# XChenZ/havatar

Hardware: AMD Instinct MI355X
Metric: rendered frames/sec @512^2, 64 samples/ray (higher is better)
Workload: dtype f32 emulated, full-width operands: every operand = hi + lo fp16 + tail (= the fp32 value itself, >= 24 significant bits); the three leading partial products on v_mfma_f32_32x32x16_f16, the three terms of order 2^-22 (hi.tail, tail.hi, lo.lo) on block-scaled 4-/6-bit v_mfma_scale_f32_32x32x64_f8f6f4

## Files before the change

### havatar_amd/csrc/hav_render.hip

```cpp
#include "hav_common.h"
#include <stdio.h>
#include <stdlib.h>
#include <string.h>
#include <atomic>

#define HAV_HID 128
#define HAV_PC 64
#define HAV_IN (2 * HAV_PC + 48)
#define KPE_STEPS 24
#define K2_STEPS (HAV_HID / 2)
#define OFF_W1PE 0
#define OFF_W2 (OFF_W1PE + KPE_STEPS * 4 * 64)
#define OFF_W4 (OFF_W2 + K2_STEPS * 4 * 64)
#define OFF_WFT (OFF_W4 + K2_STEPS * 2 * 4)
#define LDS_FLOATS (OFF_WFT + HAV_HID * 64)
#define OFF_B1 LDS_FLOATS
#define OFF_B2 (OFF_B1 + 128)
#define OFF_B4 (OFF_B2 + 128)
#define OFF_BF (OFF_B4 + 4)
#define OFF_W1F (OFF_BF + 64)
#define OFF_WFF (OFF_W1F + 2 * 128 * 64)
#define OFF_A1S (OFF_WFF + K2_STEPS * 2 * 64)
#define OFF_A2S (OFF_A1S + 3 * 4 * 3 * 64 * 4)
#define OFF_W4S (OFF_A2S + 8 * 4 * 3 * 64 * 4)
// ... 704 lines not shown
            float v[8];
            if (c < nc) getv(4 * g + c, v);
            else {
#pragma unroll
                for (int e = 0; e < 8; ++e) v[e] = 0.f;
            }
#pragma unroll
            for (int q = 0; q < 4; ++q) {
                typedef float f2 __attribute__((ext_vector_type(2)));
                typedef _Float16 h2 __attribute__((ext_vector_type(2)));
                const float v0 = v[2 * q], v1 = v[2 * q + 1];
                const h2 hi = __builtin_convertvector(f2{v0, v1}, h2);
                const uint32_t ph = __builtin_bit_cast(uint32_t, hi);
                float d0, d1;
                asm("v_fma_mix_f32 %0, %1, -1.0, %2 op_sel:[0,0,0] op_sel_hi:[1,0,0]" : "=v"(d0) : "v"(ph), "v"(v0));
                asm("v_fma_mix_f32 %0, %1, -1.0, %2 op_sel:[1,0,0] op_sel_hi:[1,0,0]" : "=v"(d1) : "v"(ph), "v"(v1));
                const h2 lo = __builtin_convertvector(f2{d0, d1}, h2);
                const uint32_t pl = __builtin_bit_cast(uint32_t, lo);
                float t0, t1;
                asm("v_fma_mix_f32 %0, %1, -1.0, %2 op_sel:[0,0,0] op_sel_hi:[1,0,0]" : "=v"(t0) : "v"(pl), "v"(d0));
                asm("v_fma_mix_f32 %0, %1, -1.0, %2 op_sel:[1,0,0] op_sel_hi:[1,0,0]" : "=v"(t1) : "v"(pl), "v"(d1));
                if (q == 0) { xh4[c].x = ph; xl4[c].x = pl; } else if (q == 1) { xh4[c].y = ph; xl4[c].y = pl; }
                else if (q == 2) { xh4[c].z = ph; xl4[c].z = pl; } else { xh4[c].w = ph; xl4[c].w = pl; }
                TB[4 * c + q] = __builtin_amdgcn_perm(__float_as_uint(t1), __float_as_uint(t0), 0x07060302u);
                if (DYN) vmax = fmaxf(vmax, fmaxf(fabsf(v0), fabsf(v1)));
            }
        }
        unsigned int E = DYN ? (__float_as_uint(vmax) >> 23) : 127u;
        if (DYN) E = E < 40u ? 40u : (E > 254u ? 254u : E);
        const unsigned int bh = E - 3u, bl = E - 13u, bt = (E - 26u) < 98u ? 98u : (E - 26u);
        const float sch = __uint_as_float(bh << 23), scl = __uint_as_float(bl << 23), sct = __uint_as_float(bt << 23);
        const int sbv = (int)(bh | (bl << 8) | (bt << 16));
        typedef _Float16 f16x16_t __attribute__((ext_vector_type(16)));
        auto cat32 = [](const uint4 (&x)[4]) {
            const f16x16_t a = __builtin_shufflevector(__builtin_bit_cast(f16x8_t, x[0]), __builtin_bit_cast(f16x8_t, x[1]), 0, 1, 2, 3, 4, 5, 6, 7, 8, 9, 10, 11, 12, 13, 14, 15);
            const f16x16_t b = __builtin_shufflevector(__builtin_bit_cast(f16x8_t, x[2]), __builtin_bit_cast(f16x8_t, x[3]), 0, 1, 2, 3, 4, 5, 6, 7, 8, 9, 10, 11, 12, 13, 14, 15);
            return __builtin_shufflevector(a, b, 0, 1, 2, 3, 4, 5, 6, 7, 8, 9, 10, 11, 12, 13, 14, 15, 16, 17, 18, 19, 20, 21, 22, 23, 24, 25, 26, 27, 28, 29, 30, 31);
        };
        const u32x6_t H6 = __builtin_amdgcn_cvt_scalef32_pk32_bf6_f16(cat32(xh4), sch);
        const u32x6_t L6 = __builtin_amdgcn_cvt_scalef32_pk32_fp6_f16(cat32(xl4), scl);
        const u32x6_t T6 = __builtin_amdgcn_cvt_scalef32_pk32_bf6_bf16(__builtin_bit_cast(bf16x32_t, TB), sct);
        const unsigned int* rec = mx + g * 4 * MX_G_DWORDS;
        u32x4_t ah[2], at[2], ala[2]; u32x2_t alb[2]; int sc[2];
        auto ldrec = [&](int slot, int m) {
            const unsigned int* r = rec + m * MX_G_DWORDS;
            ah[slot] = reinterpret_cast<const u32x4_t*>(r)[lane];
            at[slot] = reinterpret_cast<const u32x4_t*>(r + 256)[lane];
            ala[slot] = reinterpret_cast<const u32x4_t*>(r + 512)[lane];
            alb[slot] = reinterpret_cast<const u32x2_t*>(r + 768)[lane];
            sc[slot] = (int)r[896 + lane];
        };
        ldrec(0, 0);
#pragma unroll
        for (int m = 0; m < 4; ++m) {
            if (m + 1 < 4) ldrec((m + 1) & 1, m + 1);
            const int k = m & 1;
            if (HAV_MX_TERMS & 1) acc[m] = __builtin_amdgcn_mfma_scale_f32_32x32x64_f8f6f4(mx_op4(ah[k]), mx_op6(T6), acc[m], 4, 3, 0, sc[k], 2, sbv);
            if (HAV_MX_TERMS & 2) acc[m] = __builtin_amdgcn_mfma_scale_f32_32x32x64_f8f6f4(mx_op4(at[k]), mx_op6(H6), acc[m], 4, 3, 1, sc[k], 0, sbv);
            if (HAV_MX_TERMS & 4) acc[m] = __builtin_amdgcn_mfma_scale_f32_32x32x64_f8f6f4(mx_op6(ala[k], alb[k]), mx_op6(L6), acc[m], 2, 2, 2, sc[k], 1, sbv);
        }
        uint4 A[2][2];
#pragma unroll
        for (int q = 0; q < 2; ++q) A[0][q] = frag[((4 * g * 4) * 2 + q) * 64 + lane];
#pragma unroll
        for (int gg = 0; gg < 16; ++gg) {
            const int c = gg >> 2, m = gg & 3;
            if (c < nc) {
                const f16x8_t xh = __builtin_bit_cast(f16x8_t, xh4[c]), xl = __builtin_bit_cast(f16x8_t, xl4[c]);
                const f16x8_t ahh = __builtin_bit_cast(f16x8_t, A[gg & 1][0]), all_ = __builtin_bit_cast(f16x8_t, A[gg & 1][1]);
                acc[m] = __builtin_amdgcn_mfma_f32_32x32x16_f16(all_, xh, acc[m], 0, 0, 0);
                if (gg + 1 < 4 * nc) {
#pragma unroll
                    for (int q = 0; q < 2; ++q) A[(gg + 1) & 1][q] = frag[(((4 * g) * 4 + gg + 1) * 2 + q) * 64 + lane];
                }
                acc[m] = __builtin_amdgcn_mfma_f32_32x32x16_f16(ahh, xl, acc[m], 0, 0, 0);
                acc[m] = __builtin_amdgcn_mfma_f32_32x32x16_f16(ahh, xh, acc[m], 0, 0, 0);
            }
        }
    }
}

#include "hav_render_lab.h"

template <int GQ, int PREC, bool BLK, bool LEAN = false, typename Cont>
__device__ __forceinline__ void sample_eval(const MarchArgs& a_in, const LaneCtx& L, int b, float ox, float oy, float oz, float dx,
                                            float dy, float dz, float z, Cont&& cont PROF_ARG DBG_ARG)
{
    const MarchArgs& a = a_in;
    int lane = L.lane;
    asm volatile("" : "+v"(lane));
    const int h = lane >> 5;
    const float* sW1 = L.sW1;
    const float* sW2 = L.sW2;
    const float4* sW4 = L.sW4;
    int sb_off = 0;
    asm volatile("" : "+v"(sb_off));
    const float4* sBt = L.sB + sb_off;
    const int PR = a.p.plane_res, VR = a.p.vol_res;
    const float px = ox + dx * z, py = oy + dy * z, pz = oz + dz * z;
    const float* iT = a.inv_T + (size_t)b * 12;
    const float tx_ = px + iT[9], ty_ = py + iT[10], tz_ = pz + iT[11];
    const float p1x = tx_ * iT[0] + ty_ * iT[3] + tz_ * iT[6];
    const float p1y = tx_ * iT[1] + ty_ * iT[4] + tz_ * iT[7];
    const float p1z = tx_ * iT[2] + ty_ * iT[5] + tz_ * iT[8];
    float wmine;
    {
        const float gx = (h ? p1x : px) * a.p.skin_scale[0] + a.p.skin_trans[0];
        const float gy = (h ? p1y : py) * a.p.skin_scale[1] + a.p.skin_trans[1];
        const float gz = (h ? p1z : pz) * a.p.skin_scale[2] + a.p.skin_trans[2];
        const float lim = a.vlim;
        float ix = ((gx + 1.0f) * 0.5f) * lim, iy = ((gy + 1.0f) * 0.5f) * lim, iz = ((gz + 1.0f) * 0.5f) * lim;
        ix = fminf(fmaxf(ix, 0.f), lim); iy = fminf(fmaxf(iy, 0.f), lim); iz = fminf(fmaxf(iz, 0.f), lim);
        const float x0f = floorf(ix), y0f = floorf(iy), z0f = floorf(iz);
        const float fx = ix - x0f, fy = iy - y0f, fz = iz - z0f;
        const int x0 = (int)x0f, y0 = (int)y0f, z0 = (int)z0f;
        const int x1 = min(x0 + 1, VR - 1), y1 = min(y0 + 1, VR - 1), z1 = min(z0 + 1, VR - 1);
        const float* v = a.vol + (size_t)h * VR * VR * VR;
        float acc = 0.f;
#pragma unroll
        for (int cz = 0; cz < 2; ++cz)
#pragma unroll
            for (int cy = 0; cy < 2; ++cy)
#pragma unroll
                for (int cx = 0; cx < 2; ++cx) {
                    const float wgt = (cx ? fx : 1.0f - fx) * (cy ? fy : 1.0f - fy) * (cz ? fz : 1.0f - fz);
                    acc += v[((size_t)(cz ? z1 : z0) * VR + (cy ? y1 : y0)) * VR + (cx ? x1 : x0)] * wgt;
                }
        wmine = acc;
    }
    const float wother = half_swap(wmine, h);
    const float w0 = h ? wother : wmine, w1 = h ? wmine : wother;
    const float den = (w0 + w1) + 1e-8f;
    float rden = __builtin_amdgcn_rcpf(den);
    rden = rden * (2.0f - den * rden);
    float n0 = w0 * rden, n1 = w1 * rden;
    const float qx_ = n0 * px + n1 * p1x, qy_ = n0 * py + n1 * p1y, qz_ = n0 * pz + n1 * p1z;
    DBG_PUT(4, z); DBG_PUT(5, wmine); DBG_PUT(6, wother); DBG_PUT(7, (qx_ + qy_) + qz_);
    DBG_PUT(8, den); DBG_PUT(9, n0); DBG_PUT(10, n1); DBG_PUT(11, (px + py + pz) + (p1x + p1y + p1z));
    TICK(1);

    auto bias_init = [&](f32x16 (&acc1)[4]) {
#pragma unroll
        for (int m = 0; m < 4; ++m)
#pragma unroll
            for (int q = 0; q < 4; ++q) {
                if (BLK) {
                    const float4 bl = sBt[8 * m + 2 * q + h];
                    acc1[m][4 * q + 0] = bl.x; acc1[m][4 * q + 1] = bl.y; acc1[m][4 * q + 2] = bl.z; acc1[m][4 * q + 3] = bl.w;
                    continue;
                }
                const auto bb = LDB4(OFF_B1 + 32 * m + 8 * q);
                acc1[m][4 * q + 0] = __uint_as_float(bb[0]); acc1[m][4 * q + 1] = __uint_as_float(bb[1]);
                acc1[m][4 * q + 2] = __uint_as_float(bb[2]); acc1[m][4 * q + 3] = __uint_as_float(bb[3]);
            }
    };
    auto gather = [&](f32x16 (&acc1)[4]) {
        if (!ABL(1)) {
            const float lim = a.plim;
            const float gy = qy_ * a.p.nerf_scale[1] + a.p.nerf_trans[1];
            const float iy = ((gy + 1.0f) * 0.5f) * lim;
            float y0f = floorf(iy);
            const float wy1 = iy - y0f, wy0 = 1.0f - wy1;
            y0f = fminf(fmaxf(y0f, -2.f), lim + 2.f);
            const int y0 = (int)y0f, y1 = y0 + 1;
            const bool vy0 = y0 >= 0 && y0 < PR, vy1 = y1 >= 0 && y1 < PR;
            const int cy0 = min(max(y0, 0), PR - 1), cy1 = min(max(y1, 0), PR - 1);
            float tw[8];
            const float4* tp[8];
#pragma unroll
            for (int pl = 0; pl < 2; ++pl) {
                const float gx = pl ? qz_ * a.p.nerf_scale[2] + a.p.nerf_trans[2] : qx_ * a.p.nerf_scale[0] + a.p.nerf_trans[0];
                const float ix = ((gx + 1.0f) * 0.5f) * lim;
                float x0f = floorf(ix);
                const float wx1 = ix - x0f, wx0 = 1.0f - wx1;
                x0f = fminf(fmaxf(x0f, -2.f), lim + 2.f);
                const int x0 = (int)x0f, x1 = x0 + 1;
                const bool vx0 = x0 >= 0 && x0 < PR, vx1 = x1 >= 0 && x1 < PR;
                const int cx0 = min(max(x0, 0), PR - 1), cx1 = min(max(x1, 0), PR - 1);
                tw[4 * pl + 0] = (vx0 && vy0) ? wx0 * wy0 : 0.f; tw[4 * pl + 1] = (vx1 && vy0) ? wx1 * wy0 : 0.f;
                tw[4 * pl + 2] = (vx0 && vy1) ? wx0 * wy1 : 0.f; tw[4 * pl + 3] = (vx1 && vy1) ? wx1 * wy1 : 0.f;
                const int tg = pl ? HAV_TG1 : HAV_TG;
                const float* plb = a.pplanes + ((size_t)pl * a.p.B + b) * PR * PR * 128 + h * (64 << tg);
                auto texel = [&](int cy, int cx) { return reinterpret_cast<const float4*>(plb + ((size_t)((cy * PR + cx) >> tg)) * (128 << tg) + (cx & ((1 << tg) - 1)) * 4); };
                tp[4 * pl + 0] = texel(cy0, cx0);
                tp[4 * pl + 1] = texel(cy0, cx1);
                tp[4 * pl + 2] = texel(cy1, cx0);
                tp[4 * pl + 3] = texel(cy1, cx1);
            }
            if constexpr (LAB_GATHER_MODEL != 0 && PREC == 3) {
                lab_gather_model(acc1, tp, tw, lane, a.pplanes, (long long)2 * a.p.B * PR * PR * 128);
                return;
            }
            constexpr int NST = 8 * 16 / GQ;
            constexpr bool PAIRED = (GQ == 16) && HAV_TAPPAIR;
            auto tap_of = [](int g, int c) constexpr { return PAIRED ? 2 * (g >> 1) + (c & 1) : (g * GQ) / 16; };
            auto piece_of = [](int g, int c) constexpr { return PAIRED ? 8 * (g & 1) + (c >> 1) : (g * GQ) % 16 + c; };
            auto pstep = [](int tap) constexpr { return 1 << (tap >= 4 ? HAV_TG1 : HAV_TG); };
            float4 tv[2][GQ];
#pragma unroll
            for (int c = 0; c < GQ; ++c) { tv[0][c] = tp[tap_of(0, c)][pstep(tap_of(0, c)) * piece_of(0, c)]; tv[1][c] = tp[tap_of(1, c)][pstep(tap_of(1, c)) * piece_of(1, c)]; }
#pragma unroll
            for (int g = 0; g < NST; ++g) {
#pragma unroll
                for (int c = 0; c < GQ; ++c) {
                    const int c4 = piece_of(g, c);
                    const float wt = tw[tap_of(g, c)];
                    const float4 t4 = tv[g & 1][c];
                    acc1[c4 >> 2][4 * (c4 & 3) + 0] = fmaf(t4.x, wt, acc1[c4 >> 2][4 * (c4 & 3) + 0]);
                    acc1[c4 >> 2][4 * (c4 & 3) + 1] = fmaf(t4.y, wt, acc1[c4 >> 2][4 * (c4 & 3) + 1]);
                    acc1[c4 >> 2][4 * (c4 & 3) + 2] = fmaf(t4.z, wt, acc1[c4 >> 2][4 * (c4 & 3) + 2]);
                    acc1[c4 >> 2][4 * (c4 & 3) + 3] = fmaf(t4.w, wt, acc1[c4 >> 2][4 * (c4 & 3) + 3]);
                }
                asm volatile("" : "+v"(acc1[0]), "+v"(acc1[1]), "+v"(acc1[2]), "+v"(acc1[3]) : : "memory");
                if (g + 2 < NST) {
#pragma unroll
                    for (int c = 0; c < GQ; ++c) tv[g & 1][c] = tp[tap_of(g + 2, c)][pstep(tap_of(g + 2, c)) * piece_of(g + 2, c)];
                }
            }
        }
    };
    auto finish = [&](f32x16 (&acc1)[4]) {
        f32x16 acc2[4];
        float hd0, hd1, hd2, hd3;
        DBG_STAGE(0, acc1);
        TICK(2);
        float pe[KPE_STEPS];
        if (ABL(2)) {
#pragma unroll
            for (int kk = 0; kk < KPE_STEPS; ++kk) pe[kk] = qx_ * (float)(kk + 1);
        } else
#pragma unroll
        for (int kk = 0; kk < 4; ++kk) {
            const float f = h ? (float)(16 << kk) : (float)(1 << kk);
            pe_pair(qx_ * f, pe[6 * kk + 0], pe[6 * kk + 3]);
            pe_pair(qy_ * f, pe[6 * kk + 1], pe[6 * kk + 4]);
            pe_pair(qz_ * f, pe[6 * kk + 2], pe[6 * kk + 5]);
        }
        __builtin_amdgcn_sched_barrier(0);
        TICK(3);

        if (PREC == 3) {
            if (!ABL(16))
            mfma_split2x<3, false>(acc1, L.sA1, L.sMX, lane, [&](int c, float (&v)[8]) {
#pragma unroll
                for (int e = 0; e < 8; ++e) v[e] = pe[8 * c + e];
            });
        } else if (PREC == 2) {
            if (!ABL(16))
            mfma_split2h<3, 4>(acc1, L.sA1, lane, [&](int c, float (&v)[8]) {
#pragma unroll
                for (int e = 0; e < 8; ++e) v[e] = pe[8 * c + e];
            });
        } else if (PREC == 1) {
            if (!ABL(16))
            mfma_split3<3>(acc1, L.sA1, lane, [&](int c, float (&v)[8]) {
#pragma unroll
                for (int e = 0; e < 8; ++e) v[e] = pe[8 * c + e];
            });
        }
        else if (!ABL(16)) {
            float af[2][4];
#pragma unroll
            for (int m = 0; m < 4; ++m) af[0][m] = sW1[m * 64 + lane];
#pragma unroll
            for (int t = 0; t < KPE_STEPS; ++t) {
                if (t + 1 < KPE_STEPS) {
#pragma unroll
                    for (int m = 0; m < 4; ++m) af[(t + 1) & 1][m] = sW1[((t + 1) * 4 + m) * 64 + lane];
                }
#pragma unroll
                for (int m = 0; m < 4; ++m) acc1[m] = __builtin_amdgcn_mfma_f32_32x32x2f32(af[t & 1][m], pe[t], acc1[m], 0, 0, 0);
                __builtin_amdgcn_sched_barrier(0);
            }
        }
        relu_tiles<LEAN>(acc1);
        DBG_STAGE(1, acc1);
        TICK(4);

        __builtin_amdgcn_sched_barrier(0);
#pragma unroll
        for (int m = 0; m < 4; ++m)
#pragma unroll
            for (int q = 0; q < 4; ++q) {
                if (BLK) {
                    const float4 bl = sBt[32 + 8 * m + 2 * q + h];
                    acc2[m][4 * q + 0] = bl.x; acc2[m][4 * q + 1] = bl.y; acc2[m][4 * q + 2] = bl.z; acc2[m][4 * q + 3] = bl.w;
                    continue;
                }
                const auto bb = LDB4(OFF_B2 + 32 * m + 8 * q);
                acc2[m][4 * q + 0] = __uint_as_float(bb[0]); acc2[m][4 * q + 1] = __uint_as_float(bb[1]);
                acc2[m][4 * q + 2] = __uint_as_float(bb[2]); acc2[m][4 * q + 3] = __uint_as_float(bb[3]);
            }
        if (PREC == 3) {
            if (!ABL(32))
            mfma_split2x<8, true>(acc2, L.sA2, L.sMX + 4 * MX_G_DWORDS, lane, [&](int ch, float (&v)[8]) {
#pragma unroll
                for (int e = 0; e < 8; ++e) v[e] = acc1[ch >> 1][8 * (ch & 1) + e];
            });
        } else if (PREC == 2) {
            if (!ABL(32))
            mfma_split2h<8, 4>(acc2, L.sA2, lane, [&](int ch, float (&v)[8]) {
// ... 292 lines not shown
                    const float accv = racc[R_ACC];
                    float* rgb = (pass == 0 ? a.out.rgb_coarse : a.out.rgb_fine) + gr * 67;
                    rgb[3 + lane] = slot ? gb : ga;
                    if (lane < 3) {
                        float v = racc[R_RGB + lane];
                        if (a.bg) v = v + (1.0f - accv) * a.bg[gr * 3 + lane];
                        rgb[lane] = v;
                    }
                    if (lane == 0) {
                        (pass == 0 ? a.out.depth_coarse : a.out.depth_fine)[gr] = racc[R_DEPTH];
                        (pass == 0 ? a.out.acc_coarse : a.out.acc_fine)[gr] = accv;
                        if (pass == 1 || S_fp == 0) a.out.weights_max[gr] = racc[R_WMAX];
                    }
                }
            }

            if (pass == 0 && S_fp > 0 && !ABL(128)) {
                const int slot = h, li = j;
                const long long gr = (slot == 0 || has1) ? ray0 + slot : ray0;
                const RKey rkey = RANDOM ? rng_ray_key(a, gr, call_off) : RKey{0u, 0u, 0u, a.step_c};
                const float* ray = a.rays + gr * a.p.ray_stride;
                const float near = ray[6], far = ray[7];
                const int nb = S_c - 1, nw = S_c - 2, S_half = (S_c + 1) >> 1, S_f = a.p.S_f;
                float* w = s_w + slot * a.s_pad_c;
                float* cdf = s_cdf + slot * a.s_pad_c;
                float* cand = s_cand + slot * a.s_pad_f;
                float* zf = s_zf + slot * a.s_pad_f;
                if (li == 0) {
                    float sum = 0.f;
                    for (int i = 0; i < nw; ++i) sum += (w[1 + i] + 1e-5f);
                    float run = 0.f;
                    cdf[0] = 0.f;
                    for (int i = 0; i < nw; ++i) { run += (w[1 + i] + 1e-5f) / sum; cdf[i + 1] = run; }
                }
                wave_lds_sync();
                for (int k = li; k < S_f; k += 32) {
                    float u;
                    if (!RANDOM || !a.p.perturb) {
                        const float st = a.u_st;
                        u = (S_f == 1) ? 0.f : ((k < S_f / 2) ? st * (float)k : 1.0f - st * (float)(S_f - 1 - k));
                    } else {
                        const float zeta = a.u_rand ? a.u_rand[gr * S_f + k] : rng_uniform(a, rkey, k, STREAM_ZETA);
                        u = (float)k * a.u_sN + zeta * a.u_w;
                    }
                    int inds = 0;
                    for (int i = 0; i < nb; ++i) inds += (cdf[i] <= u) ? 1 : 0;
                    const int below = max(inds - 1, 0), above = min(inds, nb - 1);
                    float dnm = cdf[above] - cdf[below];
                    if (dnm < 1e-5f) dnm = 1.0f;
                    const float tt = (u - cdf[below]) / dnm;
                    const float bl = 0.5f * (z_coarse<RM>(a, gr, rkey, below + 1, near, far) + z_coarse<RM>(a, gr, rkey, below, near, far));
                    const float ba = 0.5f * (z_coarse<RM>(a, gr, rkey, above + 1, near, far) + z_coarse<RM>(a, gr, rkey, above, near, far));
                    cand[S_half + k] = bl + tt * (ba - bl);
                }
                for (int i = li; i < S_half; i += 32) cand[i] = z_coarse<RM>(a, gr, rkey, 2 * i, near, far);
                wave_lds_sync();
                for (int e = li; e < S_fp; e += 32) {
                    const float v = cand[e];
                    int rank = 0;
                    for (int q = 0; q < S_fp; ++q) {
                        const float o = cand[q];
                        rank += ((o == o) ? ((v != v) || o < v || (o == v && q < e)) : ((v != v) && q < e)) ? 1 : 0;
                    }
                    zf[rank] = v;
                    if (a.dbg_zfine && (slot == 0 || has1)) a.dbg_zfine[gr * S_fp + rank] = v;
                }
                wave_lds_sync();
            }
        }
    }
}

typedef float nt_f4 __attribute__((ext_vector_type(4)));
__device__ __forceinline__ void nt_store4(float4* p, float4 v)
{
    nt_f4 t = {v.x, v.y, v.z, v.w};
    __builtin_nontemporal_store(t, reinterpret_cast<nt_f4*>(p));
}
__device__ __forceinline__ float4 nt_load4(const float4* p)
{
    const nt_f4 t = __builtin_nontemporal_load(reinterpret_cast<const nt_f4*>(p));
    return make_float4(t.x, t.y, t.z, t.w);
}
#define HAV_GQ2 16
#define HAV_RESAMPLE_PF 8
#define HAV_LDS_BIAS 264
#define WS_H2_FLOATS 4096
#define WS_ENTRY_FLOATS (WS_H2_FLOATS + 128 + 32)
template <int RANDOM, int PREC, int CACHE>
__global__ void __launch_bounds__(MARCH_THREADS, MARCH_THREADS / 256) hav_march_blk_kernel(const MarchArgs a)
{
    constexpr int RM = RANDOM;
    constexpr bool COUT = CACHE != 2;
    constexpr bool FEATPARK = (PREC == 2) && (CACHE != 0);
    constexpr int H2F = FEATPARK ? WS_H2_FLOATS / 2 : WS_H2_FLOATS, ENTF = H2F + 128 + 32;
    if (a.guard) {
        const unsigned int unsafe = __builtin_amdgcn_readfirstlane(*a.guard);
        if ((unsafe != 0) != (a.guard_run_if != 0)) return;
        if (a.guard_run_if && a.status && blockIdx.x == 0 && threadIdx.x == 0) atomicOr(a.status, HAV_STATUS_FP16_FALLBACK);
    }
    const uint32_t call_off = RANDOM ? rng_call_off(a) : 0u;
    extern __shared__ __attribute__((aligned(16))) float smem[];
    constexpr int WLDS = PREC == 3 ? LDSX_FLOATS : (PREC == 2 ? LDSH_FLOATS : (PREC == 1 ? LDS3_FLOATS : LDS_FLOATS));
    const float* sWFF = smem + OFF_WFT;
    const int tid = threadIdx.x;
    const int lane = tid & 63;
    const int wave = __builtin_amdgcn_readfirstlane(tid >> 6);
    float* s_n = smem + WLDS + HAV_LDS_BIAS + wave * a.scr_floats;
    if (PREC == 3) {
        const float4* src = reinterpret_cast<const float4*>(a.blob + OFF_A1H);
        float4* dst = reinterpret_cast<float4*>(smem);
        for (int i = tid; i < LDSX_FP16 / 4; i += MARCH_THREADS) dst[i] = src[i];
        const float4* srcx = reinterpret_cast<const float4*>(a.blob + OFF_MX);
        float4* dstx = reinterpret_cast<float4*>(smem + LDSX_FP16);
        for (int i = tid; i < MX_GROUPS * MX_G_DWORDS / 4; i += MARCH_THREADS) dstx[i] = srcx[i];
    } else if (PREC >= 1) {
        const float4* src = reinterpret_cast<const float4*>(a.blob + (PREC == 2 ? OFF_A1H : OFF_A1S));
        float4* dst = reinterpret_cast<float4*>(smem);
        for (int i = tid; i < WLDS / 4; i += MARCH_THREADS) dst[i] = src[i];
    } else {
        const float4* src = reinterpret_cast<const float4*>(a.blob);
        float4* dst = reinterpret_cast<float4*>(smem);
        for (int i = tid; i < OFF_WFT / 4; i += MARCH_THREADS) dst[i] = src[i];
        const float4* srcf = reinterpret_cast<const float4*>(a.blob + OFF_WFF);
        float4* dstf = reinterpret_cast<float4*>(smem + OFF_WFT);
        for (int i = tid; i < K2_STEPS * 2 * 64 / 4; i += MARCH_THREADS) dstf[i] = srcf[i];
    }
    if (tid < 65) reinterpret_cast<float4*>(smem + WLDS)[tid] = reinterpret_cast<const float4*>(a.blob + OFF_B1)[tid];
    __syncthreads();

    PROF_DECL();
    PROF_BEGIN();
    const int j = lane & 31, h = lane >> 5;
    LaneCtx L;
    L.sW1 = smem + OFF_W1PE; L.sW2 = smem + OFF_W2;
    L.sW4 = reinterpret_cast<const float4*>(smem + (PREC >= 2 ? (OFF_W4H - OFF_A1H) : (PREC == 1 ? (OFF_W4S - OFF_A1S) : OFF_W4)));
    L.sA1 = reinterpret_cast<const uint4*>(smem);
    L.sA2 = reinterpret_cast<const uint4*>(smem + (PREC >= 2 ? (OFF_A2H - OFF_A1H) : (OFF_A2S - OFF_A1S)));
    L.sAF = reinterpret_cast<const uint4*>(smem + (OFF_AFH - OFF_A1H));
    L.sMX = reinterpret_cast<const unsigned int*>(smem + LDSX_FP16);
    L.sB = reinterpret_cast<const float4*>(smem + WLDS);
    L.wrs = __builtin_amdgcn_make_buffer_rsrc(const_cast<float*>(a.blob), 0, BLOB_FLOATS * 4, 0x00020000);
    L.lane = lane; L.h = h; L.hoff = h * 16;

    const int S_c = a.p.S_c, S_f = a.p.S_f, S_fp = a.S_fp, S_half = (S_c + 1) >> 1;
    const int R = a.p.R;
    const int bpf = (R + 31) >> 5;
    const long long nblk = (long long)bpf * a.p.B;

    LAB_STAGGER(wave);
    long long chunk, base, span;
    int lb, nbx;
    if ((gridDim.x & 7) == 0) {
        chunk = (nblk + 7) >> 3;
        const int xcd = blockIdx.x & 7;
        lb = blockIdx.x >> 3; nbx = gridDim.x >> 3;
        base = chunk * xcd;
        span = nblk - base; if (span > chunk) span = chunk; if (span < 0) span = 0;
    } else { base = 0; span = nblk; lb = blockIdx.x; nbx = gridDim.x; }

    for (long long local = (long long)lb * MARCH_WAVES + wave; local < span; local += (long long)nbx * MARCH_WAVES) {
        const long long blk = base + local;
        const int b = (int)(blk / bpf);
        const int r0 = (int)(blk - (long long)b * bpf) * 32 + j;
        const bool rayok = r0 < R;
        long long gr = (long long)b * R + (rayok ? r0 : R - 1);
        const float* ray = a.rays + gr * a.p.ray_stride;
// ... 34 lines not shown
        };
        auto emit = [&](int pass, const f32x16 (&hs)[4], float c0, float c1, float c2, float dep, float accw, float wmax,
                        const f32x16* fs = nullptr) {
            f32x16 og[2];
#pragma unroll
            for (int m = 0; m < 2; ++m)
#pragma unroll
                for (int q = 0; q < 4; ++q) {
                    const auto bb = __builtin_amdgcn_raw_buffer_load_b128(L.wrs, L.hoff, (OFF_BF + 32 * m + 8 * q) * 4, 0);
                    og[m][4 * q + 0] = __uint_as_float(bb[0]) * accw; og[m][4 * q + 1] = __uint_as_float(bb[1]) * accw;
                    og[m][4 * q + 2] = __uint_as_float(bb[2]) * accw; og[m][4 * q + 3] = __uint_as_float(bb[3]) * accw;
                }
            if (fs) {
#pragma unroll
                for (int m = 0; m < 2; ++m) og[m] += fs[m];
            } else if (PREC >= 1) {
                float wf[2][16];
#pragma unroll
                for (int u = 0; u < 16; ++u) wf[0][u] = __uint_as_float(__builtin_amdgcn_raw_buffer_load_b32(L.wrs, lane * 4, (OFF_WFF + u * 64) * 4, 0));
#pragma unroll
                for (int g = 0; g < 8; ++g) {
                    if (g + 1 < 8) {
#pragma unroll
                        for (int u = 0; u < 16; ++u)
                            wf[(g + 1) & 1][u] = __uint_as_float(__builtin_amdgcn_raw_buffer_load_b32(L.wrs, lane * 4, (OFF_WFF + ((g + 1) * 16 + u) * 64) * 4, 0));
                    }
#pragma unroll
                    for (int kq = 0; kq < 8; ++kq) {
                        const int ks = g * 8 + kq;
#pragma unroll
                        for (int m = 0; m < 2; ++m)
                            og[m] = __builtin_amdgcn_mfma_f32_32x32x2f32(wf[g & 1][kq * 2 + m], hs[ks >> 4][ks & 15], og[m], 0, 0, 0);
                    }
                    __builtin_amdgcn_sched_barrier(0);
                }
            } else {
#pragma unroll
                for (int ks = 0; ks < K2_STEPS; ++ks) {
#pragma unroll
                    for (int m = 0; m < 2; ++m)
                        og[m] = __builtin_amdgcn_mfma_f32_32x32x2f32(sWFF[(ks * 2 + m) * 64 + lane], hs[ks >> 4][ks & 15], og[m], 0, 0, 0);
                }
            }
            if (rayok && (pass == 1 || a.out.rgb_coarse)) {
                float* rgb = (pass == 0 ? a.out.rgb_coarse : a.out.rgb_fine) + gr * 67;
#pragma unroll
                for (int m = 0; m < 2; ++m)
#pragma unroll
                    for (int r = 0; r < 16; ++r) rgb[3 + acc_row(m, r, h)] = og[m][r];
                if (h == 0) {
                    const float bgx = a.bg ? a.bg[gr * 3 + 0] : 0.f, bgy = a.bg ? a.bg[gr * 3 + 1] : 0.f, bgz = a.bg ? a.bg[gr * 3 + 2] : 0.f;
                    rgb[0] = a.bg ? c0 + (1.0f - accw) * bgx : c0;
                    rgb[1] = a.bg ? c1 + (1.0f - accw) * bgy : c1;
                    rgb[2] = a.bg ? c2 + (1.0f - accw) * bgz : c2;
                    (pass == 0 ? a.out.depth_coarse : a.out.depth_fine)[gr] = dep;
                    (pass == 0 ? a.out.acc_coarse : a.out.acc_fine)[gr] = accw;
                    if (pass == 1 || S_fp == 0) a.out.weights_max[gr] = wmax;
                }
            }
        };

        for (int pass = 0; pass < (S_fp > 0 ? 2 : 1); ++pass) {
            const int S = pass == 0 ? S_c : S_fp;
            f32x16 hsum[4];
#pragma unroll
            for (int m = 0; m < 4; ++m)
#pragma unroll
                for (int r = 0; r < 16; ++r) hsum[m][r] = 0.f;
            float T = 1.0f, c0 = 0.f, c1 = 0.f, c2 = 0.f, dep = 0.f, accw = 0.f, wmax = 0.f;
            int ie = 0, ik = 0;
            float ze = 0.f, nk = 0.f;
            auto next_fine = [&]() -> float {
                const bool take_e = (ie < S_half) && (ik >= S_f || ze <= nk);
                const float v = take_e ? ze : nk;
                if (take_e) { ++ie; ze = (ie < S_half) ? z_coarse<RM>(a, gr, rkey, 2 * ie, near, far) : 3.0e38f; }
                else { ++ik; nk = (ik < S_f) ? s_n[ik * 32 + j] : 3.0e38f; }
                return v;
            };
            float z, znext;
            if (CACHE && pass == 1) {
                for (int k = 0; k < S_f; ++k) {
                    TICK(0);
                    const float zk = s_n[k * 32 + j];
                    sample_eval<(CACHE == 2 ? HAV_GQ2 : 8), PREC, true, CACHE == 2>(a, L, b, ox, oy, oz, dx, dy, dz, zk,
                                                                 [&](f32x16 (&acc2)[4], float hd0, float hd1, float hd2, float hd3) {
                        __builtin_amdgcn_sched_barrier(0);
                        park(S_half + k, acc2, hd0, hd1, hd2, hd3);
                    } PROF_PASS DBG_PASS(DBG_TILE(S_c + k)));
                    TICK(7);
                }
                RAY_FENCE();
                __builtin_amdgcn_fence(__ATOMIC_RELEASE, "agent");
                __builtin_amdgcn_fence(__ATOMIC_ACQUIRE, "agent");
                auto next_entry = [&](int& eid) -> float {
                    const bool take_e = (ie < S_half) && (ik >= S_f || ze <= nk);
                    const float v = take_e ? ze : nk;
                    eid = take_e ? ie : S_half + ik;
                    if (take_e) { ++ie; ze = (ie < S_half) ? z_coarse<RM>(a, gr, rkey, 2 * ie, near, far) : 3.0e38f; }
                    else { ++ik; nk = (ik < S_f) ? s_n[ik * 32 + j] : 3.0e38f; }
                    return v;
                };
                ze = z_coarse<RM>(a, gr, rkey, 0, near, far);
                nk = s_n[j];
                constexpr int FQ = 8;
                float zq[FQ]; int eq[FQ]; float4 rq[FQ];
                const float4* RAWp = reinterpret_cast<const float4*>(slot + H2F);
                int produced = 0;
#pragma unroll
                for (int u = 0; u < FQ; ++u) {
                    zq[u] = 0.f; eq[u] = 0;
                    if (produced < S) { zq[u] = next_entry(eq[u]); ++produced; }
                    rq[u] = *(&RAWp[(size_t)eq[u] * (ENTF / 4) + j]);
                }
                float dist = 0.f;
                for (int s0 = 0; s0 < S; s0 += FQ) {
#pragma unroll
                    for (int u = 0; u < FQ; ++u) {
                        const int sidx = s0 + u;
                        if (sidx < S) {
                            const float zc = zq[u];
                            const int ec = eq[u];
                            const float4 raw = rq[u];
                            if (produced < S) {
                                zq[u] = next_entry(eq[u]); ++produced;
                                rq[u] = *(&RAWp[(size_t)eq[u] * (ENTF / 4) + j]);
                            }
                            if (sidx + 1 < S) dist = zq[(u + 1) % FQ] - zc;
                            float sg = raw.w;
                            if (RANDOM && a.p.noise_std > 0.f) {
                                const float e = (RANDOM == 2 && a.noise_f) ? a.noise_f[gr * S + sidx] : rng_normal(a, rkey, gr, sidx, STREAM_EPS_F);
                                sg += e * a.p.noise_std;
                            }
                            sg = fmaxf(sg, 0.f);
                            const float alpha = 1.0f - expf(-sg * (dist * dn));
                            const float wgt = alpha * T;
                            T = T * ((1.0f - alpha) + 1e-10f);
                            c0 = fmaf(wgt, sigmoid_rcp(raw.x), c0);
                            c1 = fmaf(wgt, sigmoid_rcp(raw.y), c1);
                            c2 = fmaf(wgt, sigmoid_rcp(raw.z), c2);
                            dep = fmaf(wgt, zc, dep);
                            accw += wgt;
                            wmax = fmaxf(wmax, wgt);
                            if (h == 0) slot[(size_t)ec * ENTF + H2F + 128 + j] = wgt;
                            if (a.dbg_zfine && h == 0 && rayok) a.dbg_zfine[gr * S_fp + sidx] = zc;
                        }
                    }
                }
                TICK(0);
                RAY_FENCE();
                __builtin_amdgcn_fence(__ATOMIC_RELEASE, "agent");
                __builtin_amdgcn_fence(__ATOMIC_ACQUIRE, "agent");
                f32x16 hsumB[4];
#pragma unroll
                for (int m = 0; m < 4; ++m)
#pragma unroll
                    for (int r = 0; r < 16; ++r) hsumB[m][r] = 0.f;
                constexpr int NROW = FEATPARK ? 8 : 16;
                for (int e = 0; e < S; ++e) {
                    const float4* H2 = reinterpret_cast<const float4*>(slot + (size_t)e * ENTF);
                    const float wgt = *(&slot[(size_t)e * ENTF + H2F + 128 + j]);
#pragma unroll
                    for (int q = 0; q < NROW; ++q) {
                        const float4 v = nt_load4(&H2[q * 64 + lane]);
                        hsumB[q >> 2][4 * (q & 3) + 0] = fmaf(wgt, v.x, hsumB[q >> 2][4 * (q & 3) + 0]);
                        hsumB[q >> 2][4 * (q & 3) + 1] = fmaf(wgt, v.y, hsumB[q >> 2][4 * (q & 3) + 1]);
                        hsumB[q >> 2][4 * (q & 3) + 2] = fmaf(wgt, v.z, hsumB[q >> 2][4 * (q & 3) + 2]);
                        hsumB[q >> 2][4 * (q & 3) + 3] = fmaf(wgt, v.w, hsumB[q >> 2][4 * (q & 3) + 3]);
                    }
                }
                TICK(3);
                emit(1, hsumB, c0, c1, c2, dep, accw, wmax, FEATPARK ? hsumB : nullptr);
            }
            if (pass == 0) { z = z_coarse<RM>(a, gr, rkey, 0, near, far); znext = z_coarse<RM>(a, gr, rkey, 1, near, far); }
            else if (!CACHE) {
                ze = z_coarse<RM>(a, gr, rkey, 0, near, far);
                nk = s_n[j];
                z = next_fine(); znext = next_fine();
            }
            float dist = (CACHE && pass == 1) ? 0.f : znext - z;

            for (int s = 0; s < ((CACHE && pass == 1) ? 0 : S); ++s) {
                TICK(0);
                sample_eval<(CACHE == 2 ? HAV_GQ2 : 8), PREC, true, CACHE == 2>(a, L, b, ox, oy, oz, dx, dy, dz, z,
                                                             [&](f32x16 (&acc2)[4], float hd0, float hd1, float hd2, float hd3) {
                __builtin_amdgcn_sched_barrier(0);
                float sg = hd3;
                if (RANDOM && a.p.noise_std > 0.f) {
                    const float* nz = pass == 0 ? a.noise_c : a.noise_f;
                    const float e = (RANDOM == 2 && nz) ? nz[gr * S + s] : rng_normal(a, rkey, gr, s, pass == 0 ? STREAM_EPS_C : STREAM_EPS_F);
                    sg += e * a.p.noise_std;
                }
                sg = fmaxf(sg, 0.f);
                const float alpha = 1.0f - expf(-sg * (dist * dn));
                const float wgt = alpha * T;
                T = T * ((1.0f - alpha) + 1e-10f);
                if (COUT) {
                    const f32x16 wv = {wgt, wgt, wgt, wgt, wgt, wgt, wgt, wgt, wgt, wgt, wgt, wgt, wgt, wgt, wgt, wgt};
#pragma unroll
                    for (int m = 0; m < 4; ++m) hsum[m] = __builtin_elementwise_fma(wv, acc2[m], hsum[m]);
                }
                c0 = fmaf(wgt, sigmoid_rcp(hd0), c0);
                c1 = fmaf(wgt, sigmoid_rcp(hd1), c1);
                c2 = fmaf(wgt, sigmoid_rcp(hd2), c2);
                dep = fmaf(wgt, z, dep);
                accw += wgt;
                wmax = fmaxf(wmax, wgt);
                if (pass == 0 && S_fp > 0 && h == 0) { if (CACHE) wrow[s * 32 + j] = wgt; else if (rayok) wpark[s] = wgt; }
                if (CACHE && pass == 0 && S_fp > 0 && !(s & 1)) park(s >> 1, acc2, hd0, hd1, hd2, hd3);
                if (pass == 1 && a.dbg_zfine && h == 0 && rayok) a.dbg_zfine[gr * S_fp + s] = z;
                z = znext;
                if (s + 2 < S) {
                    znext = pass == 0 ? z_coarse<RM>(a, gr, rkey, s + 2, near, far) : next_fine();
                    dist = znext - z;
                }
                } PROF_PASS DBG_PASS(DBG_TILE(s)));
                __builtin_amdgcn_sched_barrier(0);
                TICK(7);
            }
            RAY_FENCE();

            if constexpr (CACHE != 2) {
                if (!(CACHE && pass == 1)) emit(pass, hsum, c0, c1, c2, dep, accw, wmax);
            }

            TICK(8);
            if (pass == 0 && S_fp > 0) {
                const int nw = S_c - 2, nb = S_c - 1;
                float sum = 0.f;
                constexpr int SPF = HAV_RESAMPLE_PF;
                for (int i0 = 0; i0 < nw; i0 += SPF) {
                    float t8[SPF];
#pragma unroll
                    for (int q = 0; q < SPF; ++q) t8[q] = (i0 + q < nw) ? (CACHE ? *(&wrow[(1 + i0 + q) * 32 + j]) : __builtin_nontemporal_load(&wpark[1 + i0 + q])) : 0.f;
#pragma unroll
                    for (int q = 0; q < SPF; ++q) if (i0 + q < nw) sum += (t8[q] + 1e-5f);
                }
                auto wload = [&](int i) -> float { return (i < nw) ? (CACHE ? *(&wrow[(1 + i) * 32 + j]) : __builtin_nontemporal_load(&wpark[1 + i])) : 0.f; };
                constexpr int WPF = HAV_RESAMPLE_PF;
                float wq[WPF];
#pragma unroll
                for (int q = 0; q < WPF; ++q) wq[q] = wload(q);
                float run = 0.f, cdf_lo = 0.f;
                int k = 0;
                auto u_of = [&](int kk) -> float {
                    if (!RANDOM || !a.p.perturb) {
                        const float st = a.u_st;
                        return (S_f == 1) ? 0.f : ((kk < S_f / 2) ? st * (float)kk : 1.0f - st * (float)(S_f - 1 - kk));
                    }
                    const float zeta = (RANDOM == 2 && a.u_rand) ? a.u_rand[gr * S_f + kk] : rng_uniform(a, rkey, kk, STREAM_ZETA);
                    return (float)kk * a.u_sN + zeta * a.u_w;
                };
                float u = u_of(0);
                float zi = z_coarse<RM>(a, gr, rkey, 0, near, far), zi1 = z_coarse<RM>(a, gr, rkey, 1, near, far);
                float zi2 = z_coarse<RM>(a, gr, rkey, 2, near, far);
                for (int i = 0; i < nw; ++i) {
                    const float wi = wq[0];
#pragma unroll
                    for (int q = 0; q + 1 < WPF; ++q) wq[q] = wq[q + 1];
                    wq[WPF - 1] = wload(i + WPF);
                    run += (wi + 1e-5f) / sum;
                    const float cdf_hi = run;
                    const float bl = 0.5f * (zi1 + zi), ba = 0.5f * (zi2 + zi1);
                    float dnm = cdf_hi - cdf_lo;
                    if (dnm < 1e-5f) dnm = 1.0f;
                    while (k < S_f && u < cdf_hi) {
                        const float tt = (u - cdf_lo) / dnm;
// ... 113 lines not shown
#endif
#undef BLK
static const BlkEntry* find_blk(int rm, int prec, int cm)
{
    for (const BlkEntry& e : kBlk) if (e.rm == rm && e.prec == prec && e.cm == cm) return &e;
    return nullptr;
}

extern "C" int hav_render_rays(const HavRenderParams* p, const float* rays, const float* bg, const float* inv_T,
                               const float* planes_prepared, const float* skin_vol, const void* mlp_blob, const float* t_rand,
                               const float* u_rand, const float* noise_c, const float* noise_f, const HavRenderOut* out,
                               void* stream)
{
    if (!p || !rays || !inv_T || !planes_prepared || !skin_vol || !mlp_blob || !out) return HAV_EINVAL;
    if (p->B < 1 || p->R < 0 || p->ray_stride < 8 || p->S_c < 2 || p->S_f < 0) return HAV_EINVAL;
    if (p->plane_ch != HAV_PC) return HAV_EUNSUP;
    if (p->plane_res < 2 || p->vol_res < 2) return HAV_EINVAL;
    if (p->S_c > 256 || p->S_f > 128) return HAV_EUNSUP;
    if ((p->flags & ~HAV_FLAGS_ALL) || ((p->flags & HAV_FLAG_FINE_CACHE) && (p->flags & HAV_FLAG_FINE_RECOMPUTE))) return HAV_EINVAL;
    if (p->grid_blocks < 0 || p->reserved0 != 0) return HAV_EINVAL;
    if (p->mlp_mode != HAV_MLP_SPLIT_BF16 && p->mlp_mode != HAV_MLP_F32 && p->mlp_mode != HAV_MLP_SPLIT_F16 && p->mlp_mode != HAV_MLP_SPLIT_F16_MX)
        return HAV_EINVAL;
    const bool no_coarse_out = !out->rgb_coarse && !out->depth_coarse && !out->acc_coarse;
    if (no_coarse_out ? (p->S_f <= 0) : (!out->rgb_coarse || !out->depth_coarse || !out->acc_coarse)) return HAV_EINVAL;
    if (!out->weights_max) return HAV_EINVAL;
    if (no_coarse_out && !use_block_kernel(p)) return HAV_EUNSUP;
    if (p->S_f > 0 && (!out->rgb_fine || !out->depth_fine || !out->acc_fine)) return HAV_EINVAL;
    if (p->R == 0) return 0;
    hipStream_t st = (hipStream_t)stream;

    MarchArgs a;
    a.p = *p;
    a.rays = rays; a.bg = bg; a.inv_T = inv_T; a.planes = nullptr; a.pplanes = planes_prepared; a.vol = skin_vol;
    a.blob = (const float*)mlp_blob;
    a.t_rand = t_rand; a.u_rand = u_rand; a.noise_c = noise_c; a.noise_f = noise_f;
    a.out = *out;
    a.dbg_zfine = p->dbg_zfine;
    a.ablate = env_knobs().ablate;
    a.stagger = env_knobs().stagger;
    a.guard = nullptr; a.guard_run_if = 0; a.status = p->status;
    a.ws = nullptr; a.ws_slot = 0; a.rng_base = 0;
    a.step_c = 1.0f / (float)(p->S_c - 1);
    a.u_st = p->S_f > 1 ? 1.0f / (float)(p->S_f - 1) : 0.f;
    a.u_sN = p->S_f > 0 ? (float)(1.0 / (double)p->S_f) : 0.f;
    a.u_w = p->S_f > 0 ? (float)(1.0 / (double)p->S_f - 1e-6) : 0.f;
    a.plim = (float)(p->plane_res - 1);
    a.vlim = (float)(p->vol_res - 1);
    a.NR = (long long)p->B * p->R;
    a.S_fp = p->S_f > 0 ? (p->S_c + 1) / 2 + p->S_f : 0;
    a.s_pad_c = (p->S_c + 15) & ~15;
    a.s_pad_f = ((a.S_fp > 0 ? a.S_fp : 1) + 15) & ~15;
    a.o_racc = 0;
    a.o_w = a.o_racc + 2 * RACC_N;
    a.o_cdf = a.o_w + 2 * a.s_pad_c;
    a.o_cand = a.o_cdf + 2 * a.s_pad_c;
    a.o_zf = a.o_cand + 2 * a.s_pad_f;
    a.scr_floats = (a.o_zf + 2 * a.s_pad_f + 3) & ~3;

    const bool random = p->perturb != 0 || p->noise_std > 0.f;
    static std::atomic<unsigned long long> attr_mask{0};
    int dev;
    if (!attr_done(attr_mask, dev)) {
        for (const BlkEntry& e : kBlk) {
            hipError_t er = hipFuncSetAttribute(e.fn, hipFuncAttributeMaxDynamicSharedMemorySize, 160 * 1024);
            if (er != hipSuccess) return (int)er;
        }
#ifndef HAV_FAST_BUILD
        const void* pk[2] = {(const void*)hav_march_f32_kernel<false>, (const void*)hav_march_f32_kernel<true>};
        for (int i = 0; i < 2; ++i) {
            hipError_t er = hipFuncSetAttribute(pk[i], hipFuncAttributeMaxDynamicSharedMemorySize, 160 * 1024);
            if (er != hipSuccess) return (int)er;
        }
#endif
        attr_mask.fetch_or(1ull << dev, std::memory_order_release);
    }
    const bool injected = t_rand || u_rand || noise_c || noise_f;
    const MarchVariant v = pick_variant(p, no_coarse_out, injected);
    if (v.blk) {
        a.scr_floats = ((p->S_f > 0 ? p->S_f : 1) * 32 + 3) & ~3;
        auto lds_of = [&](int prec) {
            return ((size_t)(prec == 3 ? LDSX_FLOATS : (prec == 2 ? LDSH_FLOATS : (prec == 1 ? LDS3_FLOATS : LDS_FLOATS))) + HAV_LDS_BIAS + (size_t)MARCH_WAVES * a.scr_floats) * sizeof(float);
        };
        if (lds_of(v.prec) > 160 * 1024 || (v.guard && lds_of(1) > 160 * 1024)) return HAV_EUNSUP;
        const int gridb = march_grid_blocks(p);
        const BlkEntry* main_k = find_blk(v.rm, v.prec, v.cm);
        if (!main_k) return HAV_EUNSUP;
        a.ws = v.cm ? (float*)p->workspace : nullptr;
        a.ws_slot = fine_cache_slot_floats(p);
        if (v.guard) {
            a.guard = reinterpret_cast<const unsigned int*>(planes_prepared + (size_t)2 * p->B * p->plane_res * p->plane_res * 128) + 256;
            a.guard_run_if = 0;
        }
        main_k->launch(gridb, lds_of(v.prec), st, a);
        HAV_LAUNCH_CHECK();
        if (v.guard) {
            const BlkEntry* fb = find_blk(v.rm, 1, 0);
            if (!fb) return HAV_EUNSUP;
            a.guard_run_if = 1;
            a.ws = nullptr;
            fb->launch(gridb, lds_of(1), st, a);
            HAV_LAUNCH_CHECK();
        }
    } else {
        const size_t lds = ((size_t)LDS_FLOATS + (size_t)MARCH_WAVES * a.scr_floats) * sizeof(float);
        if (lds > 160 * 1024) return HAV_EUNSUP;
        const long long npairs = (a.NR + 1) / 2;
        int grid = hav_num_cus();
        const long long need = (npairs + MARCH_WAVES - 1) / MARCH_WAVES;
        if (need < grid) grid = (int)((need + 7) / 8 * 8);
#ifndef HAV_FAST_BUILD
        if (random) hipLaunchKernelGGL(hav_march_f32_kernel<true>, dim3(grid), dim3(MARCH_THREADS), lds, st, a);
        else hipLaunchKernelGGL(hav_march_f32_kernel<false>, dim3(grid), dim3(MARCH_THREADS), lds, st, a);
#else
        (void)grid; (void)lds;
        return HAV_EUNSUP;
#endif
        HAV_LAUNCH_CHECK();
    }
    if (p->rng_counter && random) { hipLaunchKernelGGL(rng_advance_kernel, dim3(1), dim3(1), 0, st, (unsigned long long*)p->rng_counter); HAV_LAUNCH_CHECK(); }
    return 0;
}

template <int PREC, int LAYER>
__global__ void __launch_bounds__(64) debug_mlp_layer_kernel(float* __restrict__ y, const float* __restrict__ x, const float* __restrict__ blob, long long n)
{
    extern __shared__ __attribute__((aligned(16))) float smem[];
    const int lane = threadIdx.x, j = lane & 31, h = lane >> 5;
    {
        const int base = PREC == 0 ? 0 : (PREC == 1 ? OFF_A1S : OFF_A1H);
        const int cnt = PREC == 0 ? OFF_W4 : (PREC == 1 ? LDS3_FLOATS : LDSX_FP16);
        for (int i = lane; i < cnt / 4; i += 64) reinterpret_cast<float4*>(smem)[i] = reinterpret_cast<const float4*>(blob + base)[i];
        if (PREC == 3)
            for (int i = lane; i < MX_GROUPS * MX_G_DWORDS / 4; i += 64) reinterpret_cast<float4*>(smem + LDSX_FP16)[i] = reinterpret_cast<const float4*>(blob + OFF_MX)[i];
    }
    __syncthreads();
    const uint4* sA1 = reinterpret_cast<const uint4*>(smem);
    const uint4* sA2 = reinterpret_cast<const uint4*>(smem + (PREC >= 2 ? (OFF_A2H - OFF_A1H) : (OFF_A2S - OFF_A1S)));
    const unsigned int* sMX = reinterpret_cast<const unsigned int*>(smem + LDSX_FP16);
    constexpr int KIN = LAYER == 1 ? 48 : 128;
    for (long long tile = blockIdx.x; tile * 32 < n; tile += gridDim.x) {
        const long long q = tile * 32 + j;
        const long long qc = q < n ? q : n - 1;
        f32x16 acc[4], in[4];
        float pe[KPE_STEPS];
#pragma unroll
        for (int m = 0; m < 4; ++m)
#pragma unroll
            for (int r = 0; r < 16; ++r) {
                acc[m][r] = blob[(LAYER == 1 ? OFF_B1 : OFF_B2) + acc_row(m, r, h)];
                in[m][r] = LAYER == 2 ? x[qc * KIN + acc_row(m, r, h)] : 0.f;
            }
#pragma unroll
        for (int k = 0; k < KPE_STEPS; ++k) pe[k] = LAYER == 1 ? x[qc * KIN + 24 * h + k] : 0.f;
        auto get1 = [&](int c, float (&v)[8]) {
#pragma unroll
            for (int e = 0; e < 8; ++e) v[e] = pe[8 * c + e];
        };
        auto get2 = [&](int ch, float (&v)[8]) {
#pragma unroll
            for (int e = 0; e < 8; ++e) v[e] = in[ch >> 1][8 * (ch & 1) + e];
        };
        if (LAYER == 1) {
            if (PREC == 3) mfma_split2x<3, false>(acc, sA1, sMX, lane, get1);
            else if (PREC == 2) mfma_split2h<3, 4>(acc, sA1, lane, get1);
            else if (PREC == 1) mfma_split3<3>(acc, sA1, lane, get1);
            else {
// ... 83 lines not shown
```

Measured before the change: 113.3.

## Add configurable-depth gather ring with 32-bit tap offsets for lean cache path

Generalizes the triplane texel gather prefetch from a fixed double buffer to a GD-deep ring and, on the BLK+LEAN (cache mode 2) path, addresses taps via a per-plane base pointer plus 32-bit byte offsets to cut 64-bit address VGPRs. It changes the default HAV_GQ2 from 16 to 8 with ring depth 2 and uses paired tap ordering on the ring path. A guard rejects cache mode 2 when plane_res exceeds 1024 so the 32-bit offsets cannot overflow. The aim is less register pressure and better load/FMA overlap, at the cost of a different gather granularity that could reduce memory-level parallelism.

```diff
diff --git a/havatar_amd/csrc/hav_render.hip b/havatar_amd/csrc/hav_render.hip
--- a/havatar_amd/csrc/hav_render.hip
+++ b/havatar_amd/csrc/hav_render.hip
@@ -810,7 +810,7 @@
 
 #include "hav_render_lab.h"
 
-template <int GQ, int PREC, bool BLK, bool LEAN = false, typename Cont>
+template <int GQ, int PREC, bool BLK, bool LEAN = false, int GD = 2, typename Cont>
 __device__ __forceinline__ void sample_eval(const MarchArgs& a_in, const LaneCtx& L, int b, float ox, float oy, float oz, float dx,
                                             float dy, float dz, float z, Cont&& cont PROF_ARG DBG_ARG)
 {
@@ -895,6 +895,8 @@
             const int cy0 = min(max(y0, 0), PR - 1), cy1 = min(max(y1, 0), PR - 1);
             float tw[8];
             const float4* tp[8];
+            const char* pimg[2];
+            uint32_t toff[8];
 #pragma unroll
             for (int pl = 0; pl < 2; ++pl) {
                 const float gx = pl ? qz_ * a.p.nerf_scale[2] + a.p.nerf_trans[2] : qx_ * a.p.nerf_scale[0] + a.p.nerf_trans[0];
@@ -914,37 +916,61 @@
                 tp[4 * pl + 1] = texel(cy0, cx1);
                 tp[4 * pl + 2] = texel(cy1, cx0);
                 tp[4 * pl + 3] = texel(cy1, cx1);
+                pimg[pl] = reinterpret_cast<const char*>(a.pplanes + ((size_t)pl * a.p.B + b) * PR * PR * 128);
+                auto texoff = [&](int cy, int cx) { return (uint32_t)((((cy * PR + cx) >> tg) * (128 << tg) + (cx & ((1 << tg) - 1)) * 4 + h * (64 << tg)) * 4); };
+                toff[4 * pl + 0] = texoff(cy0, cx0);
+                toff[4 * pl + 1] = texoff(cy0, cx1);
+                toff[4 * pl + 2] = texoff(cy1, cx0);
+                toff[4 * pl + 3] = texoff(cy1, cx1);
             }
             if constexpr (LAB_GATHER_MODEL != 0 && PREC == 3) {
                 lab_gather_model(acc1, tp, tw, lane, a.pplanes, (long long)2 * a.p.B * PR * PR * 128);
                 return;
             }
+#define TAP_PIN() asm volatile("" : "+v"(acc1[0]), "+v"(acc1[1]), "+v"(acc1[2]), "+v"(acc1[3]) : : "memory")
+            constexpr bool RING = BLK && LEAN;
             constexpr int NST = 8 * 16 / GQ;
-            constexpr bool PAIRED = (GQ == 16) && HAV_TAPPAIR;
-            auto tap_of = [](int g, int c) constexpr { return PAIRED ? 2 * (g >> 1) + (c & 1) : (g * GQ) / 16; };
-            auto piece_of = [](int g, int c) constexpr { return PAIRED ? 8 * (g & 1) + (c >> 1) : (g * GQ) % 16 + c; };
+            constexpr bool PAIRED = (GQ == 16 || RING) && HAV_TAPPAIR;
+            constexpr int SPP = 32 / GQ;
+            static_assert(16 % GQ == 0 && GD >= 2 && GD <= NST && (RING || GD == 2), "gather stages");
+            auto tap_of = [](int g, int c) constexpr { return PAIRED ? 2 * (g / SPP) + (c & 1) : (g * GQ) / 16; };
+            auto piece_of = [](int g, int c) constexpr { return PAIRED ? (GQ / 2) * (g % SPP) + (c >> 1) : (g * GQ) % 16 + c; };
             auto pstep = [](int tap) constexpr { return 1 << (tap >= 4 ? HAV_TG1 : HAV_TG); };
-            float4 tv[2][GQ];
-#pragma unroll
-            for (int c = 0; c < GQ; ++c) { tv[0][c] = tp[tap_of(0, c)][pstep(tap_of(0, c)) * piece_of(0, c)]; tv[1][c] = tp[tap_of(1, c)][pstep(tap_of(1, c)) * piece_of(1, c)]; }
+            auto tap_ld = [&](int tap, int piece) -> float4 {
+                if (RING) return *reinterpret_cast<const float4*>(pimg[tap >> 2] + (size_t)toff[tap] + 16 * pstep(tap) * piece);
+                return tp[tap][pstep(tap) * piece];
+            };
+            float4 tv[GD][GQ];
+            if (RING) {
+#pragma unroll
+                for (int d = 0; d < GD; ++d)
+#pragma unroll
+                    for (int c = 0; c < GQ; ++c) tv[d][c] = tap_ld(tap_of(d, c), piece_of(d, c));
+                TAP_PIN();
+            } else {
+#pragma unroll
+                for (int c = 0; c < GQ; ++c) { tv[0][c] = tap_ld(tap_of(0, c), piece_of(0, c)); tv[1][c] = tap_ld(tap_of(1, c), piece_of(1, c)); }
+            }
 #pragma unroll
             for (int g = 0; g < NST; ++g) {
 #pragma unroll
                 for (int c = 0; c < GQ; ++c) {
                     const int c4 = piece_of(g, c);
                     const float wt = tw[tap_of(g, c)];
-                    const float4 t4 = tv[g & 1][c];
+                    const float4 t4 = tv[g % GD][c];
                     acc1[c4 >> 2][4 * (c4 & 3) + 0] = fmaf(t4.x, wt, acc1[c4 >> 2][4 * (c4 & 3) + 0]);
                     acc1[c4 >> 2][4 * (c4 & 3) + 1] = fmaf(t4.y, wt, acc1[c4 >> 2][4 * (c4 & 3) + 1]);
                     acc1[c4 >> 2][4 * (c4 & 3) + 2] = fmaf(t4.z, wt, acc1[c4 >> 2][4 * (c4 & 3) + 2]);
                     acc1[c4 >> 2][4 * (c4 & 3) + 3] = fmaf(t4.w, wt, acc1[c4 >> 2][4 * (c4 & 3) + 3]);
                 }
-                asm volatile("" : "+v"(acc1[0]), "+v"(acc1[1]), "+v"(acc1[2]), "+v"(acc1[3]) : : "memory");
-                if (g + 2 < NST) {
-#pragma unroll
-                    for (int c = 0; c < GQ; ++c) tv[g & 1][c] = tp[tap_of(g + 2, c)][pstep(tap_of(g + 2, c)) * piece_of(g + 2, c)];
-                }
-            }
+                TAP_PIN();
+                if (g + GD < NST) {
+#pragma unroll
+                    for (int c = 0; c < GQ; ++c) tv[g % GD][c] = tap_ld(tap_of(g + GD, c), piece_of(g + GD, c));
+                    if (RING) TAP_PIN();
+                }
+            }
+#undef TAP_PIN
         }
     };
     auto finish = [&](f32x16 (&acc1)[4]) {
@@ -1403,7 +1429,12 @@
     const nt_f4 t = __builtin_nontemporal_load(reinterpret_cast<const nt_f4*>(p));
     return make_float4(t.x, t.y, t.z, t.w);
 }
-#define HAV_GQ2 16
+#ifndef HAV_GQ2
+#define HAV_GQ2 8
+#endif
+#ifndef HAV_GD2
+#define HAV_GD2 2
+#endif
 #define HAV_RESAMPLE_PF 8
 #define HAV_LDS_BIAS 264
 #define WS_H2_FLOATS 4096
@@ -1604,7 +1635,7 @@
                 for (int k = 0; k < S_f; ++k) {
                     TICK(0);
                     const float zk = s_n[k * 32 + j];
-                    sample_eval<(CACHE == 2 ? HAV_GQ2 : 8), PREC, true, CACHE == 2>(a, L, b, ox, oy, oz, dx, dy, dz, zk,
+                    sample_eval<(CACHE == 2 ? HAV_GQ2 : 8), PREC, true, CACHE == 2, (CACHE == 2 ? HAV_GD2 : 2)>(a, L, b, ox, oy, oz, dx, dy, dz, zk,
                                                                  [&](f32x16 (&acc2)[4], float hd0, float hd1, float hd2, float hd3) {
                         __builtin_amdgcn_sched_barrier(0);
                         park(S_half + k, acc2, hd0, hd1, hd2, hd3);
@@ -1703,7 +1734,7 @@
 
             for (int s = 0; s < ((CACHE && pass == 1) ? 0 : S); ++s) {
                 TICK(0);
-                sample_eval<(CACHE == 2 ? HAV_GQ2 : 8), PREC, true, CACHE == 2>(a, L, b, ox, oy, oz, dx, dy, dz, z,
+                sample_eval<(CACHE == 2 ? HAV_GQ2 : 8), PREC, true, CACHE == 2, (CACHE == 2 ? HAV_GD2 : 2)>(a, L, b, ox, oy, oz, dx, dy, dz, z,
                                                              [&](f32x16 (&acc2)[4], float hd0, float hd1, float hd2, float hd3) {
                 __builtin_amdgcn_sched_barrier(0);
                 float sg = hd3;
@@ -1983,6 +2014,7 @@
             return ((size_t)(prec == 3 ? LDSX_FLOATS : (prec == 2 ? LDSH_FLOATS : (prec == 1 ? LDS3_FLOATS : LDS_FLOATS))) + HAV_LDS_BIAS + (size_t)MARCH_WAVES * a.scr_floats) * sizeof(float);
         };
         if (lds_of(v.prec) > 160 * 1024 || (v.guard && lds_of(1) > 160 * 1024)) return HAV_EUNSUP;
+        if (v.cm == 2 && p->plane_res > 1024) return HAV_EUNSUP;
         const int gridb = march_grid_blocks(p);
         const BlkEntry* main_k = find_blk(v.rm, v.prec, v.cm);
         if (!main_k) return HAV_EUNSUP;
```

Measured after the change: 115.2, median of 6. 1.7% higher.
